# AaronWatters/contourist

Measured on AMD Instinct MI355X. Metric: Mvoxels/s isosurface extraction on 512^3 fp32 grid, higher is better.
Workload: dtype f32

## Files before the change

### contourist_amd/csrc/cx_api.hip

```cpp
#include <cmath>
#include <cstdio>
#include <cstring>
#include <new>
#include <string>

#include "cx_ctx.h"

static int fail(cx_ctx* ctx, int code, const char* msg) {
    if (ctx) ctx->err = msg;
    return code;
}

extern "C" const char* cx_version(void) { return "contourist_hip gfx950 " __DATE__; }

extern "C" int cx_ctx_create(int device_id, cx_ctx** out) {
    if (!out) return CX_ERR_INVALID;
    *out = nullptr;
    int ndev = 0;
    if (hipGetDeviceCount(&ndev) != hipSuccess || device_id < 0 || device_id >= ndev) return CX_ERR_HIP;
    cx_ctx* ctx = new (std::nothrow) cx_ctx();
    if (!ctx) return CX_ERR_NOMEM;
    ctx->device = device_id;
    if (hipSetDevice(device_id) != hipSuccess || hipStreamCreate(&ctx->stream) != hipSuccess) {
        delete ctx;
        return CX_ERR_HIP;
    }
    ctx->own_stream = ctx->stream;
    if (ctx->counters.grow(ctx, 2048) != CX_OK ||
        hipHostMalloc(&ctx->counters_host, 2 * CX_CNT_WORDS * sizeof(uint32_t)) != hipSuccess) {
        cx_ctx_destroy(ctx);
        return CX_ERR_NOMEM;
    }
    *out = ctx;
    return CX_OK;
}

extern "C" int cx_ctx_destroy(cx_ctx* ctx) {
    if (!ctx) return CX_OK;
    (void)hipSetDevice(ctx->device);
    (void)hipDeviceSynchronize();
    cx_rccl_comm_free(ctx);
    cx_levels_free(ctx);
    cx_xfer_free(ctx);
    cx_post_free(ctx);
    cx_comp_free(ctx);
    cx_topo_free(ctx);
    cx_simplify_free(ctx);
    cx_clip_free(ctx);
    cx_cap_free(ctx);
    cx_pick_free(ctx);
    cx_state4_free(ctx);
    cx_state2_free(ctx);
    if (ctx->counters_host) (void)hipHostFree(ctx->counters_host);
    for (auto& ev : ctx->events)
        for (int n = 0; n < 5; n++)
            if (ev.e[n]) (void)hipEventDestroy(ev.e[n]);
    if (ctx->own_stream) (void)hipStreamDestroy(ctx->own_stream);
    delete ctx;
    return CX_OK;
}

extern "C" int cx_device_bytes(cx_ctx* ctx, int64_t* live_bytes, int64_t* allocations) {
    if (live_bytes) *live_bytes = ctx ? ctx->tally.live_bytes : cx_process_tally.live_bytes.load();
    if (allocations) *allocations = ctx ? ctx->tally.allocations : cx_process_tally.allocations.load();
    return CX_OK;
}

extern "C" const char* cx_last_error(cx_ctx* ctx) { return ctx ? ctx->err.c_str() : "null context"; }

extern "C" int cx_set_stream(cx_ctx* ctx, void* hip_stream) {
    if (!ctx) return CX_ERR_INVALID;
    ctx->stream = hip_stream ? (hipStream_t)hip_stream : ctx->own_stream;
    return CX_OK;
}

extern "C" int cx_synchronize(cx_ctx* ctx) {
    if (!ctx) return CX_ERR_INVALID;
    CX_HIP(ctx, hipSetDevice(ctx->device));
    CX_HIP(ctx, hipStreamSynchronize(ctx->stream));
    return CX_OK;
}

static int set_grid_dims(cx_ctx* ctx, int64_t n0, int64_t n1, int64_t n2) {
    if (n0 < 2 || n1 < 2 || n2 < 2) return fail(ctx, CX_ERR_INVALID, "grid must have at least 2 samples per axis");
    const int64_t N = n0 * n1 * n2;
    if (N > (1LL << 29)) return fail(ctx, CX_ERR_UNSUPPORTED, "more than 2^29 samples in one grid: partition into slabs");
// ... 213 lines not shown
        P.tq = nullptr; P.tlimit = 0;
        if (!fused && !typed && cx_debug_knob("CX_TQ", 0u)) {
            if ((rc = ctx->tq.grow(ctx, Z.need))) return rc;
            P.tq = ctx->tq; P.tlimit = T.wcap;
        }
        P.write_records = (!fused && !tiled && !cx_debug_knob("CX_K2_ENTRIES", 0u)) ? CX_RECORDS_SLIM : CX_RECORDS_NONE;
        if (P.write_records == CX_RECORDS_SLIM) {
            if ((rc = ctx->cbase.grow(ctx, (size_t)ctx->ccap() / 64u + 1u))) return rc;
            P.cbase = ctx->cbase;
        }
        if (tiled) {
            P.qa = nullptr;
            if ((rc = ctx->fj.grow(ctx, (size_t)P.n0 * (4u * T.njg) * P.n2 + 64u))) return rc;
            if ((rc = ctx->fk.grow(ctx, (size_t)P.n0 * P.n1 * (2u * T.nks) + 64u))) return rc;
            if ((rc = ctx->bnd.grow(ctx, (size_t)T.nblocks * 2u * T.bndcap))) return rc;
            if ((rc = ctx->bndn.grow(ctx, (size_t)T.nblocks * 2u))) return rc;
            if ((rc = ctx->torder.grow(ctx, (size_t)T.nblocks * 6u))) return rc;
            P.fj = ctx->fj; P.fk = ctx->fk; P.bnd = ctx->bnd; P.bndn = ctx->bndn; P.torder = ctx->torder;
            P.tile_cap = cx_debug_knob("CX_TILE_CAP", cx_tile_cap_default());
        }
        P.nvw = cx_vertex_stage_waves(P);
        if ((rc = ctx->rstart.grow(ctx, (size_t)P.nvw + 1u))) return rc;
        P.rstart = ctx->rstart;
        P.nkw = cx_triangle_stage_waves(P);
        if ((rc = ctx->kstart.grow(ctx, (size_t)P.nkw + 1u))) return rc;
        P.kstart = ctx->kstart;
        ctx->last = P;
    }
    ctx->last_task = T;
    ctx->last_flags = flags;
    ctx->path = staged ? (fused ? 2 : (tiled ? 3 : 1)) : 0;
    ctx->records_valid = staged ? (P.write_records == CX_RECORDS_FULL) : true;
    cx_ctx::evset* ev = nullptr;
    if (ctx->timing && ctx->nevents < (int)(sizeof(ctx->events) / sizeof(ctx->events[0])) && ctx->events[ctx->nevents].e[4])
        ev = &ctx->events[ctx->nevents++];
    if (!staged)
        CX_HIP(ctx, hipMemsetAsync(ctx->counters, 0, CX_CNT_WORDS * sizeof(uint32_t), ctx->stream));
    if (ev) CX_HIP(ctx, hipEventRecord(ev->e[0], ctx->stream));
    if (staged) {
        cx_launch_stream(P, T, ctx->stream);
        if (ev) CX_HIP(ctx, hipEventRecord(ev->e[1], ctx->stream));
        cx_launch_scan_waves(P, T, ctx->stream);
        if (ev) CX_HIP(ctx, hipEventRecord(ev->e[2], ctx->stream));
        if (fused) cx_launch_emit_mesh(P, T, ctx->stream);
        else if (tiled) cx_launch_tile_emit(P, T, ctx->hash_xy, ctx->stream);
        else cx_launch_emit_vertices(P, T, ctx->stream);
    } else {
        cx_launch_classify_generic(P, ctx->stream);
        if (ev) CX_HIP(ctx, hipEventRecord(ev->e[1], ctx->stream));
        if (ev) CX_HIP(ctx, hipEventRecord(ev->e[2], ctx->stream));
    }
    if (ev) CX_HIP(ctx, hipEventRecord(ev->e[3], ctx->stream));
    if (!fused && !tiled) {
        if (staged && P.write_records) cx_launch_emit_triangles_q(P, T, ctx->hash_xy, ctx->stream);
        else if (staged) cx_launch_emit_triangles_e(P, T, ctx->hash_xy, ctx->stream);
        else cx_launch_emit_triangles(P, ctx->hash_xy, ctx->stream);
    }
    if (ev) CX_HIP(ctx, hipEventRecord(ev->e[4], ctx->stream));
    CX_HIP(ctx, hipGetLastError());
    ctx->extracted = true;
    ctx->counts_fetched = false;
    ctx->post_valid = false;
    ctx->keep_valid = false;
    ctx->cap_valid = false;
    cx_levels_invalidate(ctx);
    return CX_OK;
}

// ... 170 lines not shown
    hipLaunchKernelGGL(cx_k_read_bw, dim3(256 * 8), dim3(256), 0, ctx->stream, static_cast<const uint4*>(device_ptr), n16, sink);
    CX_HIP(ctx, hipGetLastError());
    double best = 0.0;
    const uint32_t grids[3] = {256u * 8u, 256u * 16u, 256u * 32u};
    for (int r = 0; r < reps; r++)
        for (uint32_t g : grids) {
            CX_HIP(ctx, hipEventRecord(e0, ctx->stream));
            hipLaunchKernelGGL(cx_k_read_bw, dim3(g), dim3(256), 0, ctx->stream, static_cast<const uint4*>(device_ptr), n16, sink);
            CX_HIP(ctx, hipGetLastError());
            CX_HIP(ctx, hipEventRecord(e1, ctx->stream));
            CX_HIP(ctx, hipEventSynchronize(e1));
            float ms = 0.f;
            CX_HIP(ctx, hipEventElapsedTime(&ms, e0, e1));
            if (ms > 0.f) best = fmax(best, (double)n16 * 16.0 / (ms * 1e-3) / 1e9);
        }
    *out_GBps = best;
    return CX_OK;
}
extern "C" int cx_measure_read_bandwidth(cx_ctx* ctx, const void* device_ptr, int64_t bytes, int reps, double* out_GBps) {
    if (!ctx || !device_ptr || bytes < (1 << 20) || reps < 1 || !out_GBps) return ctx ? fail(ctx, CX_ERR_INVALID, "cx_measure_read_bandwidth: bad argument") : CX_ERR_INVALID;
    CX_HIP(ctx, hipSetDevice(ctx->device));
    if (!ctx->counters) return fail(ctx, CX_ERR_STATE, "context has no scratch words yet (extract once first)");
    cx_buf<uint32_t> sink;
    hipEvent_t e0 = nullptr, e1 = nullptr;
    int rc = sink.grow(ctx, 256);
    if (!rc && (hipEventCreate(&e0) != hipSuccess || hipEventCreate(&e1) != hipSuccess)) rc = fail(ctx, CX_ERR_HIP, "cx_measure_read_bandwidth: hipEventCreate failed");
    if (!rc) rc = read_bandwidth(ctx, device_ptr, (size_t)bytes / 16u, reps, e0, e1, sink, out_GBps);
    if (rc) (void)hipStreamSynchronize(ctx->stream);
    if (e0) (void)hipEventDestroy(e0);
    if (e1) (void)hipEventDestroy(e1);
    return rc;
}

extern "C" int cx_timing_enable(cx_ctx* ctx, int on) {
    if (!ctx) return CX_ERR_INVALID;
    ctx->nevents = 0;
    ctx->timing = false;
    if (!on) return CX_OK;
    CX_HIP(ctx, hipSetDevice(ctx->device));
    for (auto& ev : ctx->events)
        for (int n = 0; n < 5; n++)
            if (!ev.e[n]) CX_HIP(ctx, hipEventCreateWithFlags(&ev.e[n], hipEventDisableSystemFence));
    ctx->timing = true;
    return CX_OK;
}

extern "C" int cx_timing_read(cx_ctx* ctx, double ms[8], int* n) {
    if (!ctx || !ms) return CX_ERR_INVALID;
    CX_HIP(ctx, hipSetDevice(ctx->device));
    CX_HIP(ctx, hipStreamSynchronize(ctx->stream));
    for (int k = 0; k < 8; k++) ms[k] = 0.0;
    for (int i = 0; i < ctx->nevents; i++) {
        float d[4] = {0, 0, 0, 0};
        for (int k = 0; k < 4; k++) CX_HIP(ctx, hipEventElapsedTime(&d[k], ctx->events[i].e[k], ctx->events[i].e[k + 1]));
        ms[0] += d[0] + d[1] + d[2]; ms[1] += d[3]; ms[2] += d[0] + d[1] + d[2] + d[3];
        ms[3] += d[0]; ms[4] += d[1]; ms[5] += d[2];
    }
    if (n) *n = ctx->nevents;
    ctx->nevents = 0;
    return CX_OK;
}
```

### contourist_amd/csrc/cx_common.h

```cpp
#pragma once
#include <hip/hip_runtime.h>
#include <stdint.h>

#include <type_traits>

#include "../../include/contourist_hip.h"
#include "cx_tables.h"

#include <cstdlib>
#include <cstring>
static inline bool cx_debug_enabled() {
    static const bool on = [] { const char* e = getenv("CX_DEBUG"); return e && strcmp(e, "1") == 0; }();
    return on;
}
static inline uint32_t cx_debug_knob(const char* name, uint32_t dflt) {
    if (!cx_debug_enabled()) return dflt;
    const char* e = getenv(name);
    return (e && atoi(e) > 0) ? (uint32_t)atoi(e) : dflt;
}

struct cx_fdiv {
    uint32_t mul, sh1, sh2, d;
};

// ... 39 lines not shown
template <> struct cx_dt<CX_DTYPE_U8> : cx_dt_int<CX_DTYPE_U8, uint8_t> {};
template <> struct cx_dt<CX_DTYPE_I8> : cx_dt_int<CX_DTYPE_I8, int8_t> {};
template <> struct cx_dt<CX_DTYPE_U16> : cx_dt_int<CX_DTYPE_U16, uint16_t> {};
template <> struct cx_dt<CX_DTYPE_I16> : cx_dt_int<CX_DTYPE_I16, int16_t> {};
template <> struct cx_dt<CX_DTYPE_F16> : cx_dt_narrow<CX_DTYPE_F16, uint16_t, uint16_t> {
    static __device__ __forceinline__ float cvt(uint32_t v) { return (float)__builtin_bit_cast(_Float16, (uint16_t)v); }
};
template <> struct cx_dt<CX_DTYPE_BF16> : cx_dt_narrow<CX_DTYPE_BF16, uint16_t, uint16_t> {
    static __device__ __forceinline__ float cvt(uint32_t v) { return __uint_as_float(v << 16); }
};
template <int DT>
__device__ __forceinline__ const typename cx_dt<DT>::T* cx_grid_data(const cx_grid_ref& g) {
    return static_cast<const typename cx_dt<DT>::T*>(g.p);
}
template <int DT>
__device__ __forceinline__ float cx_sample(const cx_grid_ref& g, size_t i) {
    if constexpr (DT == CX_DTYPE_F32) return cx_grid_data<DT>(g)[i];
    else return cx_dt<DT>::cvt((uint32_t)(typename cx_dt<DT>::bits)cx_grid_data<DT>(g)[i]);
}
static inline size_t cx_dtype_size(int32_t dt) {
    return dt == CX_DTYPE_F32 ? 4u : (dt == CX_DTYPE_U8 || dt == CX_DTYPE_I8) ? 1u : 2u;
}
static inline bool cx_dtype_valid(int32_t dt) { return dt >= CX_DTYPE_F32 && dt <= CX_DTYPE_BF16; }
#define CX_DISPATCH_DTYPE(dt, F)                                   \
    switch (dt) {                                                  \
        case CX_DTYPE_U8: F(CX_DTYPE_U8); break;                   \
        case CX_DTYPE_I8: F(CX_DTYPE_I8); break;                   \
        case CX_DTYPE_U16: F(CX_DTYPE_U16); break;                 \
        case CX_DTYPE_I16: F(CX_DTYPE_I16); break;                 \
        case CX_DTYPE_F16: F(CX_DTYPE_F16); break;                 \
        case CX_DTYPE_BF16: F(CX_DTYPE_BF16); break;               \
        default: F(CX_DTYPE_F32); break;                           \
    }

struct cx_params {
    cx_grid_ref grid;
    uint32_t n0, n1, n2;
    uint32_t nsamples;
    cx_fdiv div_plane;
    cx_fdiv div_row;
    float vcmp;
    float near_abs;
    float vhi, vlo;
    double value;
    double tol_value;
    uint32_t flags;
    uint32_t org0, org1, org2;
    uint64_t* celltab;
    cx_vrec* verts;
    uint4* cells;
    int32_t* tris;
    uint32_t vcap, ccap, tcap;
    uint32_t* counters;
    unsigned long long* stamps;
    uint32_t* queue;
    struct cx_brec* brec;
    struct cx_wsum* wsum;
    struct cx_wbase* wbase;
    struct cx_bdesc* flat;
    uint32_t fcap;
    uint32_t* qa;
    uint32_t* info;
    const uint8_t* hbytes;
    uint64_t* info64;
    cx_fdiv div_ci;
    uint32_t* chunksum;
    uint32_t fused;
    uint32_t* rstart;
    uint32_t nvw;
    uint32_t qlimit;
    uint32_t* kstart;
    uint32_t nkw;
    uint32_t write_records;
    uint32_t records_only;
    uint2* cbase;
    float* tq;
    uint32_t tlimit;
    uint64_t* fj;
    uint64_t* fk;
    uint4* bnd;
    uint32_t* bndn;
    uint32_t* torder;
    uint32_t tile_cap;
};
enum { CX_RECORDS_NONE = 0, CX_RECORDS_FULL = 1, CX_RECORDS_SLIM = 2 };
#ifndef CX_SWP
#define CX_SWP 16u
#endif

struct cx_wsum {
    uint32_t nb;
    uint32_t v, t, c, b;
    uint32_t nq;
    uint32_t near;
    uint32_t nr;
};
struct cx_wbase {
    uint32_t v, t, c, boff;
};
struct cx_brec {
    uint32_t qoff, n, vpre, tpre, cpre, near, pad0, pad1;
};

struct cx_bdesc {
    uint32_t w;
    uint32_t qofs, n;
    uint32_t vbase, tbase, cbase;
    uint32_t near;
    uint32_t rbase;
    uint32_t p, j0, k0;
    uint32_t nsteps;
};

struct cx_task {
    uint32_t ci;
    uint32_t nks, njg, nic;
// ... 41 lines not shown
```

### contourist_amd/csrc/cx_ctx.h

```cpp
#pragma once
#include <atomic>
#include <string>
#include <type_traits>
#include <utility>

#include "cx_common.h"

#define CX_HIP(ctx, call)                                                                        \
    do {                                                                                         \
        hipError_t e__ = (call);                                                                 \
        if (e__ != hipSuccess) {                                                                 \
            (ctx)->err = std::string(#call) + ": " + hipGetErrorString(e__);                     \
            return (e__ == hipErrorOutOfMemory) ? CX_ERR_NOMEM : CX_ERR_HIP;                      \
        }                                                                                        \
    } while (0)

static inline uint32_t cx_blocks(size_t n, uint32_t b = 256) { return (uint32_t)((n + b - 1) / b); }
static inline dim3 cx_grid1(size_t n) { return dim3(n ? cx_blocks(n) : 1u); }
static inline unsigned long long cx_table_size(size_t n) {
    unsigned long long s = 1024;
    while (s < 2 * (unsigned long long)n + 16) s <<= 1;
    return s;
}

// ... 103 lines not shown
    cx_buf<uint32_t> counters;
    uint32_t* counters_host = nullptr;
    bool extracted = false;
    bool counts_fetched = false;
    cx_counts counts = {0, 0, 0, 0};
    cx_params last;
    cx_buf<uint8_t> tri_keep;
    cx_buf<uint8_t> seed_buf[8];
    int seed_mode = 0;
    bool keep_valid = false;
    cx_buf<float4> attr_n0;
    cx_buf<double> attr_n1;
    cx_buf<float> attr_v0;
    cx_buf<double> attr_v1;
    cx_buf<uint8_t> attr_e1;
    cx_buf<uint8_t> attr_grid;
    cx_buf<float4> attr_c0;
    cx_buf<double> attr_c1;
    struct cx_comp_state* comp = nullptr;
    struct cx_simplify_state* simp = nullptr;
    struct cx_topo_state* topo = nullptr;
    struct cx_clip_state* clip = nullptr;
    struct cx_cap_state* cap = nullptr;
    bool cap_valid = false;
    struct cx_pick_state* pick = nullptr;
    cx_post_state* post = nullptr;
    bool post_valid = false;
    cx_buf<unsigned long long> stamps;
    void* rccl_comm = nullptr;
    bool rccl_owned = true;
    int rccl_rank = 0, rccl_world = 1;
    void* xfer_stage[2] = {nullptr, nullptr};
    hipEvent_t xfer_ev[2] = {nullptr, nullptr};
    struct evset { hipEvent_t e[5] = {nullptr, nullptr, nullptr, nullptr, nullptr}; };
    bool timing = false;
    int nevents = 0;
    evset events[256];
};

template <typename T>
int cx_buf<T>::fail(cx_ctx* ctx, size_t bytes, hipError_t e) {
    ctx->err = std::string("device buffer (") + std::to_string(bytes) + " bytes): " + hipGetErrorString(e);
    return (e == hipErrorOutOfMemory) ? CX_ERR_NOMEM : CX_ERR_HIP;
}
template <typename T>
hipError_t cx_buf<T>::alloc(cx_ctx* ctx, size_t n) {
    void* fresh = nullptr;
    const hipError_t e = hipMalloc(&fresh, n * sizeof(T));
    if (e != hipSuccess) return e;
    p_ = static_cast<T*>(fresh); cap_ = n; tally_ = &ctx->tally;
    tally_->live_bytes += (int64_t)bytes(); tally_->allocations++;
    cx_process_tally.live_bytes += (int64_t)bytes(); cx_process_tally.allocations++;
    return hipSuccess;
}
template <typename T>
int cx_buf<T>::grow(cx_ctx* ctx, size_t need) {
    if (cap_ >= need && p_) return CX_OK;
    if (need == 0) return CX_OK;
    hipError_t e = hipStreamSynchronize(ctx->stream);
    if (e == hipSuccess && p_) e = hipFree(p_);
    forget();
    if (e == hipSuccess) e = alloc(ctx, need);
    return e == hipSuccess ? CX_OK : fail(ctx, need * sizeof(T), e);
}
template <typename T>
int cx_buf<T>::grow_keep(cx_ctx* ctx, size_t used, size_t need) {
    if (cap_ >= need && p_) return CX_OK;
    if (need == 0) return CX_OK;
    const size_t want = need > cap_ + cap_ / 2 ? need : cap_ + cap_ / 2;
    cx_buf fresh;
// ... 101 lines not shown
```

### contourist_amd/csrc/cx_stream3d.h

```cpp
#pragma once

__device__ __forceinline__ uint32_t cx_task_of_block(const cx_task& T) {
    return (blockIdx.x & 7u) * T.chunk + (blockIdx.x >> 3);
}
struct cx_tile {
    uint32_t k0, j0, p, ib, nrows;
};
__device__ __forceinline__ cx_tile cx_tile_of(const cx_params& P, const cx_task& T, uint32_t b, uint32_t wave) {
    cx_tile t;
    const uint32_t ks = b % T.nks; b /= T.nks;
    const uint32_t jg = b % T.njg;
    const uint32_t ic = b / T.njg;
    t.k0 = ks * 256u;
    t.j0 = jg * (4u * CX_RJ) + wave * CX_RJ;
    t.p = ic * T.ci;
    t.ib = min(t.p + T.ci, P.n0);
    t.nrows = (t.j0 < P.n1) ? min((uint32_t)CX_RJ, P.n1 - t.j0) : 0u;
    return t;
}

#define CX_SQ 512u
#define CX_PLW 260u
#define CX_SBR 32u
static_assert((CX_SWP - 1u) * 1024u / CX_BATCH_MIN + 1u <= CX_SBR, "a streaming wave can close more batches than its LDS stage holds");
static_assert(CX_SQ >= 512u, "half a wave's lanes queue up to 512 cells per step");
template <int DT> struct cx_row4 { typedef float4 v; typedef float h; };
template <> struct cx_row4<CX_DTYPE_U8> { typedef uint32_t v; typedef uint32_t h; };
template <> struct cx_row4<CX_DTYPE_I8> { typedef uint32_t v; typedef uint32_t h; };
template <> struct cx_row4<CX_DTYPE_U16> { typedef cx_v2u v; typedef uint32_t h; };
template <> struct cx_row4<CX_DTYPE_I16> { typedef cx_v2u v; typedef uint32_t h; };
template <> struct cx_row4<CX_DTYPE_F16> { typedef cx_v2u v; typedef uint32_t h; };
template <> struct cx_row4<CX_DTYPE_BF16> { typedef cx_v2u v; typedef uint32_t h; };
template <typename V, size_t AL>
struct __attribute__((packed, aligned(AL))) cx_row4_ua { V v; };
template <int DT>
__device__ __forceinline__ void cx_row4_unpack(const typename cx_row4<DT>::v& w, float& x, float& y, float& z, float& t) {
    if constexpr (sizeof(typename cx_dt<DT>::T) == 1) {
        x = cx_dt<DT>::cvt(w); y = cx_dt<DT>::cvt(w >> 8); z = cx_dt<DT>::cvt(w >> 16); t = cx_dt<DT>::cvt(w >> 24);
    } else {
        x = cx_dt<DT>::cvt(w.x); y = cx_dt<DT>::cvt(w.x >> 16); z = cx_dt<DT>::cvt(w.y); t = cx_dt<DT>::cvt(w.y >> 16);
    }
}
template <bool ALIGNED, int DT>
__device__ __forceinline__ void cx_stream_tile(const cx_params& P, const cx_task& T, const uint32_t b) {
    __shared__ uint32_t s_q[4][CX_SQ];
    __shared__ uint32_t s_br[4][CX_SBR][5];
    extern __shared__ __attribute__((aligned(16))) float s_pl_dyn[];
    __shared__ uint32_t s_tot[4][8];
    __shared__ uint8_t s_ntri[256];
    if (b >= T.nblocks) return;
    s_ntri[threadIdx.x] = cx_d_voxel_ntri[threadIdx.x];
    if (b == 0u && threadIdx.x < 3u && P.torder) P.counters[CX_CNT_TCLS + threadIdx.x] = 0u;
    __syncthreads();
    const uint32_t lane = cx_lane_id();
    const uint32_t wave = __builtin_amdgcn_readfirstlane(threadIdx.x >> 6);
    uint32_t* q = s_q[wave];
    uint32_t ql = 0, qflushed = 0;
    uint32_t nbl = 0, nbflushed = 0;
    const uint32_t w = b * 4u + wave;
    unsigned long long* stamp = P.stamps ? P.stamps + (size_t)w * 4u : nullptr;
    if (stamp && lane == 0) stamp[0] = __builtin_amdgcn_s_memtime();
    const cx_tile tile = cx_tile_of(P, T, b, wave);
    const uint32_t k0 = tile.k0, j0 = tile.j0, ib = tile.ib, nrows = tile.nrows;
    uint32_t p = tile.p;
    uint32_t* __restrict__ gq = P.queue + (size_t)w * T.wcap;
    cx_brec* __restrict__ brec = P.brec + (size_t)w * T.bcap;
    const typename cx_dt<DT>::bits* __restrict__ A = reinterpret_cast<const typename cx_dt<DT>::bits*>(cx_grid_data<DT>(P.grid));
    cx_cnt acc = {0, 0, 0, 0};
    uint32_t qn = 0, qstart = 0, nb = 0;
    uint32_t rv = 0, rt = 0, rc = 0;
    uint32_t nr = 0;
    uint32_t tv = 0;
    bool overflow_t = false;
    float dnear = 3.0e38f;
    cx_fast_geom G;
    G.pstart = p; G.j0 = j0; G.k0 = k0;
    bool overflow = false;
// ... 241 lines not shown
    if (near && qn != 0u && !overflow) {
        __threadfence();
        cx_run ex = {0, 0, 0, 0, 0};
        cx_process_queue<false, DT>(P, [&](uint32_t x) { return cx_entry_lin(P, G, __builtin_nontemporal_load(gq + x)); }, qn, lane, false, ex, nullptr);
        really_near = !(ex.v == rv && ex.t == rt && ex.c == rc && ex.s == 0u);
        run.b = ex.b;
        if (really_near) { run.v = ex.v; run.t = ex.t; run.c = ex.c; }
    }
    if (overflow_t && qn != 0u && !overflow) really_near = true;
    if (really_near) {
        nb = 1;
        nr = (qn + 63u) >> 6;
        if (lane == 0) {
            cx_brec R;
            R.qoff = 0; R.n = qn; R.vpre = 0; R.tpre = 0; R.cpre = 0; R.near = 1; R.pad0 = 0; R.pad1 = 0;
            brec[0] = R;
        }
    }
    if (lane == 0) {
        cx_wsum S;
        S.nb = nb; S.v = run.v; S.t = run.t; S.c = run.c; S.b = run.b; S.nq = qn; S.near = really_near ? 1u : 0u; S.nr = nr;
        P.wsum[w] = S;
        s_tot[wave][0] = run.v; s_tot[wave][1] = run.t; s_tot[wave][2] = run.c; s_tot[wave][3] = run.b; s_tot[wave][4] = nb;
        s_tot[wave][5] = (really_near && qn != 0u) ? 1u : 0u;
        s_tot[wave][6] = nr;
        s_tot[wave][7] = overflow ? 1u : 0u;
    }
    __syncthreads();
    if (threadIdx.x < 8u) {
        const uint32_t sum = s_tot[0][threadIdx.x] + s_tot[1][threadIdx.x] + s_tot[2][threadIdx.x] + s_tot[3][threadIdx.x];
        uint32_t* cs = P.chunksum + (size_t)(b >> 6) * 8u;
        if (sum) atomicAdd(cs + threadIdx.x, sum);
    }
}
template <bool ALIGNED, int DT>
__global__ __launch_bounds__(256, CX_K1_MIN_WAVES) void cx_k_stream(const cx_params P, const cx_task T) {
    cx_stream_tile<ALIGNED, DT>(P, T, cx_task_of_block(T));
}
#define CX_LEVELS_PER_LAUNCH 8u
struct cx_params_pack {
    cx_params p[CX_LEVELS_PER_LAUNCH];
};
template <bool ALIGNED, int DT>
__global__ __launch_bounds__(256, CX_K1_MIN_WAVES) void cx_k_stream_levels(const cx_params_pack LP, const cx_task T, const uint32_t nlevels) {
    const uint32_t seq = blockIdx.x >> 3;
    const uint32_t tile_seq = seq / nlevels, level = seq - tile_seq * nlevels;
    cx_stream_tile<ALIGNED, DT>(LP.p[level], T, (blockIdx.x & 7u) * T.chunk + tile_seq);
}

__device__ __forceinline__ void cx_scan_list_chunk(const cx_params& P, const cx_task& T, const uint32_t nw, const uint32_t g, const uint32_t nchunks) {
    __shared__ uint32_t s_part[4][8];
    __shared__ uint32_t s_own[4][6];
    const uint32_t tid = threadIdx.x, lane = cx_lane_id(), wave = tid >> 6;
    uint32_t acc[6] = {0, 0, 0, 0, 0, 0}, near_any = 0, rall = 0, over_any = 0;
    for (uint32_t c = tid; c < nchunks; c += 256u) {
        const uint4 lo = *reinterpret_cast<const uint4*>(P.chunksum + (size_t)c * 8u);
        const uint4 hi = *reinterpret_cast<const uint4*>(P.chunksum + (size_t)c * 8u + 4u);
        if (c < g) { acc[0] += lo.x; acc[1] += lo.y; acc[2] += lo.z; acc[3] += lo.w; acc[4] += hi.x; acc[5] += hi.z; }
        near_any |= hi.y;
        rall += hi.z;
        over_any |= hi.w;
    }
    const uint32_t w = g * 256u + tid;
    cx_wsum S;
    S.nb = S.v = S.t = S.c = S.b = S.nq = S.near = S.nr = 0;
    if (w < nw) S = P.wsum[w];
    near_any |= (S.near != 0u && S.nq != 0u) ? 1u : 0u;
    const uint32_t x[6] = {S.v, S.t, S.c, S.b, S.nb, S.nr};
    uint32_t inc[6];
#pragma unroll
    for (int m = 0; m < 6; m++) {
        inc[m] = cx_wave_incl_scan(x[m], lane);
        const uint32_t before = cxd_wave_add(acc[m]);
        if (lane == 63u) { s_own[wave][m] = inc[m]; s_part[wave][m] = before; }
    }
    {
        const uint32_t nr = (__ballot(near_any != 0u) != 0ULL) ? 1u : 0u;
        const uint32_t ra = cxd_wave_add(rall);
        const uint32_t ov = (__ballot(over_any != 0u) != 0ULL) ? 1u : 0u;
        if (lane == 63u) { s_part[wave][6] = nr | (ov << 1); s_part[wave][7] = ra; }
// ... 37 lines not shown
        uint32_t rank = 0;
#pragma unroll
        for (uint32_t c = 0; c < 3u; c++) {
            const uint64_t m = __ballot(cls == c);
            if (cls == c) rank = cx_mbcnt(m);
            if (lane == 0) s_cls[c][wave] = (uint32_t)__popcll(m);
        }
        __syncthreads();
        if (tid < 3u) {
            const uint32_t n = s_cls[tid][0] + s_cls[tid][1] + s_cls[tid][2] + s_cls[tid][3];
            s_clsbase[tid] = n ? atomicAdd(&P.counters[CX_CNT_TCLS + tid], n) : 0u;
        }
        __syncthreads();
        if (cls < 3u) {
            uint32_t at = s_clsbase[cls] + rank;
            for (uint32_t ww = 0; ww < wave; ww++) at += s_cls[cls][ww];
            P.torder[(size_t)cls * (nw >> 1) + at] = w >> 1;
        } else if (cls == 3u) {
            P.bndn[w >> 1] = 0u;
        }
    }
    if (g == nchunks - 1u && tid == 255u) {
        P.counters[CX_CNT_VERTS] = ex[0] + x[0]; P.counters[CX_CNT_TRIS] = ex[1] + x[1];
        P.counters[CX_CNT_CELLS] = ex[2] + x[2]; P.counters[CX_CNT_BORDER] = ex[3] + x[3];
        P.counters[CX_CNT_BATCHES] = ex[4] + x[4];
        P.counters[CX_CNT_ROUNDS] = rounds;
        const uint32_t fl = s_part[0][6] | s_part[1][6] | s_part[2][6] | s_part[3][6];
        P.counters[CX_CNT_NEAR] = fl & 1u;
        P.counters[CX_CNT_OVERFLOW] = (fl >> 1) & 1u;
        P.counters[CX_CNT_TILEOVF] = 0u;
    }
}
__global__ __launch_bounds__(256) void cx_k_scan_list(const cx_params P, const cx_task T, const uint32_t nw) {
    cx_scan_list_chunk(P, T, nw, blockIdx.x, gridDim.x);
}
__global__ __launch_bounds__(256) void cx_k_scan_list_levels(const cx_params* __restrict__ LP, const cx_task T, const uint32_t nw) {
    const cx_params P = LP[blockIdx.y];
    cx_scan_list_chunk(P, T, nw, blockIdx.x, gridDim.x);
}
```

### contourist_amd/csrc/cx_tri3d.h

```cpp
#pragma once

#define CX_PY_P1 11400714785074694791ULL
#define CX_PY_P2 14029467366897019727ULL
#define CX_PY_P5 2870177450012600261ULL
__device__ __forceinline__ uint64_t py_round(uint64_t acc, uint32_t x) {
    acc += (uint64_t)x * CX_PY_P2;
    acc = (acc << 31) | (acc >> 33);
    return acc * CX_PY_P1;
}
__device__ __forceinline__ uint64_t py_round_signed(uint64_t acc, int32_t x) {
    const uint64_t lane = (x == -1) ? ~1ULL : (uint64_t)(int64_t)x;
    acc += lane * CX_PY_P2;
    acc = (acc << 31) | (acc >> 33);
    return acc * CX_PY_P1;
}
__device__ __forceinline__ uint64_t py_round_tail(uint64_t acc) {
    acc = (acc << 31) | (acc >> 33);
    return acc * CX_PY_P1;
}
__device__ __forceinline__ uint64_t py_finish3(uint64_t acc) {
    acc += 3ULL ^ (CX_PY_P5 ^ 3527539ULL);
    return (acc == ~0ULL) ? 1546275796ULL : acc;
}
__global__ void cx_k_hash_xy(uint64_t* table, uint32_t n0, uint32_t n1, uint32_t org0, uint32_t org1) {
// ... 459 lines not shown
    for (uint32_t c = 0; c < 6; c++) {
        uint2 pr = make_uint2(0u, 0u);
        if ((A.geo >> c) & 1u) {
            const uint32_t qa = A.qa[c];
            const uint32_t below = qa & ((1u << bit[c]) - 1u);
            const uint32_t at = qb[c] + (qa >> 16) + __popc(below);
            const uint64_t e = P.info64[at];
            pr = make_uint2((uint32_t)e, (uint32_t)(e >> 32));
        }
        I.nb[c] = pr;
    }
    I.ck = A.ck;
    I.hb[0] = I.hb[1] = I.hb[2] = I.hb[3] = 0;
    I.hxy[0] = I.hxy[1] = I.hxy[2] = I.hxy[3] = 0;
    const uint32_t sm = A.rec.y & 0xFFu, tetskip = (A.rec.y >> 8) & 0x3Fu, ntri = (A.rec.y >> 16) & 0xFFu;
    if ((P.flags & CX_DIAG_CPYTHON310) && cx_need_hash(sm, tetskip, ntri) != 0u) {
        struct __attribute__((packed, aligned(8))) u64x2 { uint64_t a, b; };
        const u64x2 p0 = *reinterpret_cast<const u64x2*>(hash_xy + A.ij);
        const u64x2 p1 = *reinterpret_cast<const u64x2*>(hash_xy + (A.ij + P.n1));
        I.hxy[0] = p0.a; I.hxy[1] = p0.b; I.hxy[2] = p1.a; I.hxy[3] = p1.b;
    }
}
__device__ __forceinline__ void cx_triq_pin2(cx_tri_in& I) {
    asm volatile("" : "+v"(I.hxy[0]), "+v"(I.hxy[1]), "+v"(I.hxy[2]), "+v"(I.hxy[3]) :: "memory");
    asm volatile("" : "+v"(I.nb[0].x), "+v"(I.nb[0].y), "+v"(I.nb[1].x), "+v"(I.nb[1].y), "+v"(I.nb[2].x), "+v"(I.nb[2].y) :: "memory");
    asm volatile("" : "+v"(I.nb[3].x), "+v"(I.nb[3].y), "+v"(I.nb[4].x), "+v"(I.nb[4].y), "+v"(I.nb[5].x), "+v"(I.nb[5].y) :: "memory");
}
#ifndef CX_K2Q_MIN_WAVES
#define CX_K2Q_MIN_WAVES 5
#endif
template <bool NEG_ORIGIN, bool SLIM>
__global__ __launch_bounds__(256, CX_K2Q_MIN_WAVES) void cx_k_emit_triangles_q(const cx_params P, const cx_task T, const uint64_t* __restrict__ hash_xy) {
    __shared__ cx_tri_lds L;
    const uint32_t ncells = min(P.counters[CX_CNT_CELLS], P.ccap);
    if (P.counters[CX_CNT_TRIS] > P.tcap || P.counters[CX_CNT_VERTS] > P.vcap) return;
    if (SLIM && P.counters[CX_CNT_CELLS] > P.ccap) return;
    if (blockIdx.x * blockDim.x >= ncells) return;
    cx_tri_lds_init(L);
    __syncthreads();
    const uint32_t lane = cx_lane_id();
    const uint32_t wave = __builtin_amdgcn_readfirstlane(threadIdx.x >> 6);
    const uint32_t stride = gridDim.x * blockDim.x;
    uint32_t idx = blockIdx.x * blockDim.x + threadIdx.x;
    const uint4 zero = make_uint4(0, 0, 0, 0);
    auto record = [&](uint32_t at) {
        const uint32_t c = min(at, ncells - 1u);
        if constexpr (SLIM) {
            const uint2 r = cx_load_record2(reinterpret_cast<const uint2*>(P.cells) + c);
            const uint2 b = P.cbase[__builtin_amdgcn_readfirstlane(c >> 6)];
            return make_uint4(r.x, r.y, b.x, b.y);
        } else {
            return cx_load_record(P.cells + c);
        }
    };
    auto valid = [&](const uint4& r, uint32_t at) { return (at < ncells) ? r : zero; };
    cx_tri_qa Ab, Ac;
    cx_tri_in Ia, Ib;
    uint4 rec_c = record(idx + 2u * stride);
    {
        uint4 r0 = record(idx), r1 = record(idx + stride);
        asm volatile("" : "+v"(r0.x), "+v"(r0.y), "+v"(r0.z), "+v"(r0.w), "+v"(r1.x), "+v"(r1.y), "+v"(r1.z), "+v"(r1.w) :: "memory");
        cx_triq_stage1(P, T, L, valid(r0, idx), Ac);
        cx_triq_stage1(P, T, L, valid(r1, idx + stride), Ab);
        cx_triq_pin1(Ac, rec_c);
        cx_triq_pin1(Ab, rec_c);
        cx_triq_stage2(P, T, hash_xy, Ac, Ia);
        cx_triq_pin2(Ia);
    }
    while (idx - lane < ncells) {
        const uint32_t nidx = idx + stride;
        uint4 rec_d = record(nidx + 2u * stride);
        cx_triq_stage1(P, T, L, valid(rec_c, nidx + stride), Ac);
        cx_triq_stage2(P, T, hash_xy, Ab, Ib);
        const uint32_t ttot = cx_tri_phase1<NEG_ORIGIN, SLIM>(P, L, lane, wave, Ia);
        cx_tri_phase2(P, L, lane, wave, ttot);
        cx_triq_pin1(Ac, rec_d);
        cx_triq_pin2(Ib);
        Ia = Ib;
        Ab = Ac;
        rec_c = rec_d;
        idx = nidx;
    }
}

__device__ __forceinline__ cx_bdesc cx_desc_uniform(const cx_bdesc& D) {
    cx_bdesc U;
    U.w = __builtin_amdgcn_readfirstlane(D.w); U.qofs = __builtin_amdgcn_readfirstlane(D.qofs); U.n = __builtin_amdgcn_readfirstlane(D.n);
    U.vbase = 0; U.cbase = 0; U.p = 0; U.j0 = 0; U.k0 = 0; U.nsteps = 0;
    U.tbase = __builtin_amdgcn_readfirstlane(D.tbase);
    U.near = __builtin_amdgcn_readfirstlane(D.near); U.rbase = __builtin_amdgcn_readfirstlane(D.rbase);
    return U;
}
struct cx_esrc {
    uint32_t f, nbatches, lo, hi;
    uint32_t at, bend;
    uint32_t qofs, w;
    uint32_t bend_round;
    uint32_t tbase;
    cx_bdesc next;
    bool done;
};
__device__ __forceinline__ void cx_esrc_enter(const cx_params& P, cx_esrc& S, const cx_bdesc& Draw) {
    const cx_bdesc D = cx_desc_uniform(Draw);
    const uint32_t nrb = (D.n + 63u) >> 6;
    const uint32_t r0 = max(S.lo, D.rbase) - D.rbase, r1 = min(S.hi, D.rbase + nrb) - D.rbase;
    S.qofs = D.qofs; S.w = D.w; S.bend_round = D.rbase + nrb; S.tbase = D.tbase;
    if (D.near) { S.at = 0u; S.bend = (r0 == 0u) ? D.n : 0u; }
    else { S.at = r0 * 64u; S.bend = min(D.n, r1 * 64u); }
    if (S.f + 1u < S.nbatches) S.next = P.flat[S.f + 1u];
}
__device__ __forceinline__ void cx_esrc_advance(const cx_params& P, cx_esrc& S) {
    while (S.at >= S.bend && !S.done) {
        if (S.bend_round >= S.hi || S.f + 1u >= S.nbatches) { S.done = true; break; }
        S.f++;
        cx_esrc_enter(P, S, S.next);
// ... 114 lines not shown
```

### contourist_amd/csrc/cx_vertex3d.h

```cpp
#pragma once

__device__ __forceinline__ void cx_skip_rounds(const cx_params& P, const cx_fast_geom& G, const uint32_t* q, uint32_t rounds, uint32_t lane,
                                               const uint8_t* ntri_lut, cx_run& run) {
    uint32_t v = 0, t = 0, c = 0;
    for (uint32_t r = 0; r < rounds; r++) {
        const uint32_t e = q[r * 64u + lane];
        uint32_t i, j, k;
        cx_decode_entry(P, G, e, i, j, k);
        const uint32_t vm = cx_corner_valid(P, i, j, k);
        const uint32_t sm = cx_entry_signs(e);
        const uint32_t s0 = (sm & 1u) ? 0xFFu : 0u;
        const uint32_t nv = __popc(((sm ^ s0) & vm) & 0xFEu);
        const uint32_t nt = (vm == 0xFFu) ? (uint32_t)ntri_lut[sm] : 0u;
        v += nv; t += nt; c += (nv | nt) ? 1u : 0u;
    }
    run.v += cxd_wave_add(v); run.t += cxd_wave_add(t); run.c += cxd_wave_add(c);
}

#ifndef CX_S3_MIN_WAVES
#define CX_S3_MIN_WAVES 1
#endif
template <bool TQ, int DT>
__global__ __launch_bounds__(256, CX_S3_MIN_WAVES) void cx_k_emit_vertices(const cx_params P, const cx_task T) {
    __shared__ float4 s_vstage[4][CX_VSTAGE_LDS];
    __shared__ uint8_t s_ntri[256];
    s_ntri[threadIdx.x] = cx_d_voxel_ntri[threadIdx.x];
    __syncthreads();
    const uint32_t lane = cx_lane_id();
    const uint32_t wave = __builtin_amdgcn_readfirstlane(threadIdx.x >> 6);
    const uint32_t nbatches = min(P.counters[CX_CNT_BATCHES], P.fcap);
    const uint32_t rounds = P.counters[CX_CNT_ROUNDS];
    const uint32_t nvw = gridDim.x * 4u;
    const uint32_t share = max((rounds + nvw - 1u) / nvw, CX_S3_MIN_SHARE);
    const uint32_t lo = (blockIdx.x * 4u + wave) * share;
    if (lo >= rounds || nbatches == 0u) return;
    const uint32_t hi = min(rounds, lo + share);
    uint32_t f = P.rstart[blockIdx.x * 4u + wave];
    if (f >= nbatches) return;
    cx_bdesc D = P.flat[f];
    for (;;) {
        const uint32_t fn = f + 1u;
        cx_bdesc Dn = D;
        if (fn < nbatches) Dn = P.flat[fn];
        const uint32_t nrb = (D.n + 63u) >> 6;
        const uint32_t r0 = max(lo, D.rbase) - D.rbase, r1 = min(hi, D.rbase + nrb) - D.rbase;
        cx_fast_geom G;
        G.pstart = D.p; G.j0 = D.j0; G.k0 = D.k0;
        const uint32_t* __restrict__ q = P.queue + D.qofs;
        cx_run run;
        run.v = D.vbase; run.t = D.tbase; run.c = D.cbase; run.b = 0;
        uint64_t* __restrict__ info = P.info64 + D.qofs;
        if (!D.near) {
            if (r0) cx_skip_rounds(P, G, q, r0, lane, s_ntri, run);
            if (TQ)
                cx_emit_queue_t(P, G, q, r0 * 64u, min(D.n, r1 * 64u), lane, run, reinterpret_cast<uint32_t*>(s_vstage[wave]), s_ntri, info,
                                reinterpret_cast<const uint32_t*>(P.tq) + ((size_t)D.w * T.wcap) - __builtin_amdgcn_readfirstlane(P.wbase[D.w].v));
            else
                cx_emit_queue_fast<DT>(P, G, q, r0 * 64u, min(D.n, r1 * 64u), lane, run, reinterpret_cast<uint32_t*>(s_vstage[wave]), s_ntri, info);
        } else if (r0 == 0u) {
            cx_process_queue<true, DT>(P, [&](uint32_t x) { return cx_entry_lin(P, G, q[x]); }, D.n, lane, true, run, reinterpret_cast<cx_vrec*>(s_vstage[wave]), info);
        }
        if (D.rbase + nrb >= hi || fn >= nbatches) break;
        f = fn;
        D = Dn;
    }
}
```

Measured before the change: 440,700.

## Time kernels with in-kernel realtime stamps and use scalar loads for vertex setup

After: 440,700 (median of 2 runs). No clear change (+0.0%).

```diff
diff --git a/contourist_amd/csrc/cx_api.hip b/contourist_amd/csrc/cx_api.hip
--- a/contourist_amd/csrc/cx_api.hip
+++ b/contourist_amd/csrc/cx_api.hip
@@ -52,6 +52,7 @@
     cx_state4_free(ctx);
     cx_state2_free(ctx);
     if (ctx->counters_host) (void)hipHostFree(ctx->counters_host);
+    if (ctx->tslots_host) (void)hipHostFree(ctx->tslots_host);
     for (auto& ev : ctx->events)
         for (int n = 0; n < 5; n++)
             if (ev.e[n]) (void)hipEventDestroy(ev.e[n]);
@@ -331,8 +332,13 @@
     ctx->path = staged ? (fused ? 2 : (tiled ? 3 : 1)) : 0;
     ctx->records_valid = staged ? (P.write_records == CX_RECORDS_FULL) : true;
     cx_ctx::evset* ev = nullptr;
-    if (ctx->timing && ctx->nevents < (int)(sizeof(ctx->events) / sizeof(ctx->events[0])) && ctx->events[ctx->nevents].e[4])
-        ev = &ctx->events[ctx->nevents++];
+    if (ctx->timing && ctx->nevents < (int)cx_ctx::CX_TIMED_MAX && ctx->tslots && ctx->events[ctx->nevents].e[4]) {
+        const bool stamped = staged && P.write_records == CX_RECORDS_SLIM && !cx_debug_knob("CX_TIMING_EVENTS", 0u);
+        const int i = ctx->nevents++;
+        ctx->by_events[i] = !stamped;
+        if (stamped) P.tslots = ctx->tslots + (size_t)i * CX_TS_KERNELS;
+        else ev = &ctx->events[i];
+    }
     if (!staged)
         CX_HIP(ctx, hipMemsetAsync(ctx->counters, 0, CX_CNT_WORDS * sizeof(uint32_t), ctx->stream));
     if (ev) CX_HIP(ctx, hipEventRecord(ev->e[0], ctx->stream));
@@ -569,12 +575,32 @@
     return rc;
 }
 
+static int timing_clear_used(cx_ctx* ctx) {
+    if (ctx->nevents > 0 && ctx->tslots)
+        CX_HIP(ctx, hipMemsetAsync(ctx->tslots, 0, (size_t)ctx->nevents * CX_TS_KERNELS * sizeof(cx_tslot), ctx->stream));
+    ctx->nevents = 0;
+    return CX_OK;
+}
+
 extern "C" int cx_timing_enable(cx_ctx* ctx, int on) {
     if (!ctx) return CX_ERR_INVALID;
-    ctx->nevents = 0;
+    CX_HIP(ctx, hipSetDevice(ctx->device));
     ctx->timing = false;
+    {
+        const int rc = timing_clear_used(ctx);
+        if (rc) return rc;
+    }
     if (!on) return CX_OK;
-    CX_HIP(ctx, hipSetDevice(ctx->device));
+    if (!ctx->tslots) {
+        const size_t nslots = (size_t)cx_ctx::CX_TIMED_MAX * CX_TS_KERNELS;
+        const int rc = ctx->tslots.grow(ctx, nslots);
+        if (rc) return rc;
+        CX_HIP(ctx, hipMemsetAsync(ctx->tslots, 0, ctx->tslots.bytes(), ctx->stream));
+        CX_HIP(ctx, hipHostMalloc(&ctx->tslots_host, nslots * sizeof(cx_tslot)));
+        int khz = 0;
+        if (hipDeviceGetAttribute(&khz, hipDeviceAttributeWallClockRate, ctx->device) != hipSuccess || khz <= 0) khz = 100000;
+        ctx->ticks_per_ms = (double)khz;
+    }
     for (auto& ev : ctx->events)
         for (int n = 0; n < 5; n++)
             if (!ev.e[n]) CX_HIP(ctx, hipEventCreateWithFlags(&ev.e[n], hipEventDisableSystemFence));
@@ -582,18 +608,39 @@
     return CX_OK;
 }
 
+static double stamp_ms(const cx_tslot& S, double ticks_per_ms) {
+    unsigned long long end = 0ULL;
+    for (uint32_t k = 0; k < CX_TS_ENDS; k++) end = S.end[k] > end ? S.end[k] : end;
+    if (S.start == 0ULL || end <= S.start) return 0.0;
+    return (double)(end - S.start) / ticks_per_ms;
+}
+
 extern "C" int cx_timing_read(cx_ctx* ctx, double ms[8], int* n) {
     if (!ctx || !ms) return CX_ERR_INVALID;
     CX_HIP(ctx, hipSetDevice(ctx->device));
     CX_HIP(ctx, hipStreamSynchronize(ctx->stream));
     for (int k = 0; k < 8; k++) ms[k] = 0.0;
+    bool stamps = false;
+    for (int i = 0; i < ctx->nevents; i++) stamps = stamps || !ctx->by_events[i];
+    if (stamps) {
+        CX_HIP(ctx, hipMemcpyAsync(ctx->tslots_host, ctx->tslots, (size_t)ctx->nevents * CX_TS_KERNELS * sizeof(cx_tslot), hipMemcpyDeviceToHost, ctx->stream));
+        CX_HIP(ctx, hipStreamSynchronize(ctx->stream));
+    }
     for (int i = 0; i < ctx->nevents; i++) {
-        float d[4] = {0, 0, 0, 0};
-        for (int k = 0; k < 4; k++) CX_HIP(ctx, hipEventElapsedTime(&d[k], ctx->events[i].e[k], ctx->events[i].e[k + 1]));
-        ms[0] += d[0] + d[1] + d[2]; ms[1] += d[3]; ms[2] += d[0] + d[1] + d[2] + d[3];
-        ms[3] += d[0]; ms[4] += d[1]; ms[5] += d[2];
-    }
+        double d[4] = {0, 0, 0, 0};
+        if (ctx->by_events[i]) {
+            float e[4] = {0, 0, 0, 0};
+            for (int k = 0; k < 4; k++) CX_HIP(ctx, hipEventElapsedTime(&e[k], ctx->events[i].e[k], ctx->events[i].e[k + 1]));
+            for (int k = 0; k < 4; k++) d[k] = e[k];
+        } else {
+            const cx_tslot* S = ctx->tslots_host + (size_t)i * CX_TS_KERNELS;
+            d[0] = stamp_ms(S[CX_TS_STREAM], ctx->ticks_per_ms); d[1] = stamp_ms(S[CX_TS_SCAN], ctx->ticks_per_ms);
+            d[2] = stamp_ms(S[CX_TS_VERTS], ctx->ticks_per_ms); d[3] = stamp_ms(S[CX_TS_TRIS], ctx->ticks_per_ms);
+        }
+        ms[3] += d[0]; ms[4] += d[1]; ms[5] += d[2]; ms[1] += d[3];
+    }
+    ms[0] = ms[3] + ms[4] + ms[5];
+    ms[2] = ms[0] + ms[1];
     if (n) *n = ctx->nevents;
-    ctx->nevents = 0;
-    return CX_OK;
-}
+    return timing_clear_used(ctx);
+}
diff --git a/contourist_amd/csrc/cx_common.h b/contourist_amd/csrc/cx_common.h
--- a/contourist_amd/csrc/cx_common.h
+++ b/contourist_amd/csrc/cx_common.h
@@ -95,6 +95,41 @@
         case CX_DTYPE_BF16: F(CX_DTYPE_BF16); break;               \
         default: F(CX_DTYPE_F32); break;                           \
     }
+
+#define CX_TS_ENDS 32u
+struct cx_tslot {
+    unsigned long long start;
+    unsigned long long end[CX_TS_ENDS];
+};
+enum { CX_TS_STREAM = 0, CX_TS_SCAN = 1, CX_TS_VERTS = 2, CX_TS_TRIS = 3, CX_TS_KERNELS = 4 };
+typedef unsigned long long cx_ts_stash[2];
+__device__ __forceinline__ void cx_ts_begin(cx_tslot* ts, uint32_t k, unsigned long long* stash) {
+    unsigned long long end = 0ULL, t0 = 0ULL;
+    if (ts) {
+        end = (unsigned long long)reinterpret_cast<uintptr_t>(&ts[k].end[blockIdx.x & (CX_TS_ENDS - 1u)]);
+        if (blockIdx.x == 0u) t0 = __builtin_amdgcn_s_memrealtime();
+    }
+    if (threadIdx.x == 0u) { stash[0] = end; stash[1] = t0; }
+}
+__device__ __forceinline__ void cx_ts_end(const unsigned long long* stash) {
+    if (!stash || (threadIdx.x & 63u) != 0u) return;
+    typedef __attribute__((address_space(1))) unsigned long long gu64;
+    gu64* const end = reinterpret_cast<gu64*>((uintptr_t)stash[0]);
+    if (!end) return;
+    __hip_atomic_fetch_max(end, (unsigned long long)__builtin_amdgcn_s_memrealtime(), __ATOMIC_RELAXED, __HIP_MEMORY_SCOPE_AGENT);
+    if (threadIdx.x == 0u && stash[1] != 0ULL) end[-1] = stash[1];
+}
+template <typename T>
+__device__ __forceinline__ T cx_ro(const T* p) {
+    static_assert(sizeof(T) % 4u == 0u && std::is_trivially_copyable<T>::value, "words");
+    const __attribute__((address_space(4))) uint32_t* q = (const __attribute__((address_space(4))) uint32_t*)(p);
+    uint32_t w[sizeof(T) / 4u];
+#pragma unroll
+    for (uint32_t k = 0; k < sizeof(T) / 4u; k++) w[k] = q[k];
+    T v;
+    __builtin_memcpy(&v, w, sizeof(T));
+    return v;
+}
 
 struct cx_params {
     cx_grid_ref grid;
@@ -145,6 +180,7 @@
     uint32_t* bndn;
     uint32_t* torder;
     uint32_t tile_cap;
+    cx_tslot* tslots;
 };
 enum { CX_RECORDS_NONE = 0, CX_RECORDS_FULL = 1, CX_RECORDS_SLIM = 2 };
 #ifndef CX_SWP
diff --git a/contourist_amd/csrc/cx_ctx.h b/contourist_amd/csrc/cx_ctx.h
--- a/contourist_amd/csrc/cx_ctx.h
+++ b/contourist_amd/csrc/cx_ctx.h
@@ -159,10 +159,15 @@
     int rccl_rank = 0, rccl_world = 1;
     void* xfer_stage[2] = {nullptr, nullptr};
     hipEvent_t xfer_ev[2] = {nullptr, nullptr};
+    enum { CX_TIMED_MAX = 256 };
     struct evset { hipEvent_t e[5] = {nullptr, nullptr, nullptr, nullptr, nullptr}; };
     bool timing = false;
     int nevents = 0;
-    evset events[256];
+    evset events[CX_TIMED_MAX];
+    bool by_events[CX_TIMED_MAX] = {};
+    cx_buf<cx_tslot> tslots;
+    cx_tslot* tslots_host = nullptr;
+    double ticks_per_ms = 1.0e5;
 };
 
 template <typename T>
diff --git a/contourist_amd/csrc/cx_stream3d.h b/contourist_amd/csrc/cx_stream3d.h
--- a/contourist_amd/csrc/cx_stream3d.h
+++ b/contourist_amd/csrc/cx_stream3d.h
@@ -42,7 +42,7 @@
     }
 }
 template <bool ALIGNED, int DT>
-__device__ __forceinline__ void cx_stream_tile(const cx_params& P, const cx_task& T, const uint32_t b) {
+__device__ __forceinline__ void cx_stream_tile(const cx_params& P, const cx_task& T, const uint32_t b, const unsigned long long* ts_stash) {
     __shared__ uint32_t s_q[4][CX_SQ];
     __shared__ uint32_t s_br[4][CX_SBR][5];
     extern __shared__ __attribute__((aligned(16))) float s_pl_dyn[];
@@ -350,10 +350,13 @@
         uint32_t* cs = P.chunksum + (size_t)(b >> 6) * 8u;
         if (sum) atomicAdd(cs + threadIdx.x, sum);
     }
+    cx_ts_end(ts_stash);
 }
 template <bool ALIGNED, int DT>
 __global__ __launch_bounds__(256, CX_K1_MIN_WAVES) void cx_k_stream(const cx_params P, const cx_task T) {
-    cx_stream_tile<ALIGNED, DT>(P, T, cx_task_of_block(T));
+    __shared__ cx_ts_stash s_ts;
+    cx_ts_begin(P.tslots, CX_TS_STREAM, s_ts);
+    cx_stream_tile<ALIGNED, DT>(P, T, cx_task_of_block(T), s_ts);
 }
 #define CX_LEVELS_PER_LAUNCH 8u
 struct cx_params_pack {
@@ -363,7 +366,7 @@
 __global__ __launch_bounds__(256, CX_K1_MIN_WAVES) void cx_k_stream_levels(const cx_params_pack LP, const cx_task T, const uint32_t nlevels) {
     const uint32_t seq = blockIdx.x >> 3;
     const uint32_t tile_seq = seq / nlevels, level = seq - tile_seq * nlevels;
-    cx_stream_tile<ALIGNED, DT>(LP.p[level], T, (blockIdx.x & 7u) * T.chunk + tile_seq);
+    cx_stream_tile<ALIGNED, DT>(LP.p[level], T, (blockIdx.x & 7u) * T.chunk + tile_seq, nullptr);
 }
 
 __device__ __forceinline__ void cx_scan_list_chunk(const cx_params& P, const cx_task& T, const uint32_t nw, const uint32_t g, const uint32_t nchunks) {
@@ -467,7 +470,10 @@
     }
 }
 __global__ __launch_bounds__(256) void cx_k_scan_list(const cx_params P, const cx_task T, const uint32_t nw) {
+    __shared__ cx_ts_stash s_ts;
+    cx_ts_begin(P.tslots, CX_TS_SCAN, s_ts);
     cx_scan_list_chunk(P, T, nw, blockIdx.x, gridDim.x);
+    cx_ts_end(s_ts);
 }
 __global__ __launch_bounds__(256) void cx_k_scan_list_levels(const cx_params* __restrict__ LP, const cx_task T, const uint32_t nw) {
     const cx_params P = LP[blockIdx.y];
diff --git a/contourist_amd/csrc/cx_tri3d.h b/contourist_amd/csrc/cx_tri3d.h
--- a/contourist_amd/csrc/cx_tri3d.h
+++ b/contourist_amd/csrc/cx_tri3d.h
@@ -515,6 +515,8 @@
 template <bool NEG_ORIGIN, bool SLIM>
 __global__ __launch_bounds__(256, CX_K2Q_MIN_WAVES) void cx_k_emit_triangles_q(const cx_params P, const cx_task T, const uint64_t* __restrict__ hash_xy) {
     __shared__ cx_tri_lds L;
+    __shared__ cx_ts_stash s_ts;
+    cx_ts_begin(P.tslots, CX_TS_TRIS, s_ts);
     const uint32_t ncells = min(P.counters[CX_CNT_CELLS], P.ccap);
     if (P.counters[CX_CNT_TRIS] > P.tcap || P.counters[CX_CNT_VERTS] > P.vcap) return;
     if (SLIM && P.counters[CX_CNT_CELLS] > P.ccap) return;
@@ -564,6 +566,7 @@
         rec_c = rec_d;
         idx = nidx;
     }
+    cx_ts_end(s_ts);
 }
 
 __device__ __forceinline__ cx_bdesc cx_desc_uniform(const cx_bdesc& D) {
diff --git a/contourist_amd/csrc/cx_vertex3d.h b/contourist_amd/csrc/cx_vertex3d.h
--- a/contourist_amd/csrc/cx_vertex3d.h
+++ b/contourist_amd/csrc/cx_vertex3d.h
@@ -24,20 +24,22 @@
 __global__ __launch_bounds__(256, CX_S3_MIN_WAVES) void cx_k_emit_vertices(const cx_params P, const cx_task T) {
     __shared__ float4 s_vstage[4][CX_VSTAGE_LDS];
     __shared__ uint8_t s_ntri[256];
+    __shared__ cx_ts_stash s_ts;
+    cx_ts_begin(P.tslots, CX_TS_VERTS, s_ts);
     s_ntri[threadIdx.x] = cx_d_voxel_ntri[threadIdx.x];
     __syncthreads();
     const uint32_t lane = cx_lane_id();
     const uint32_t wave = __builtin_amdgcn_readfirstlane(threadIdx.x >> 6);
-    const uint32_t nbatches = min(P.counters[CX_CNT_BATCHES], P.fcap);
-    const uint32_t rounds = P.counters[CX_CNT_ROUNDS];
+    const uint32_t nbatches = min(cx_ro(P.counters + CX_CNT_BATCHES), P.fcap);
+    const uint32_t rounds = cx_ro(P.counters + CX_CNT_ROUNDS);
     const uint32_t nvw = gridDim.x * 4u;
     const uint32_t share = max((rounds + nvw - 1u) / nvw, CX_S3_MIN_SHARE);
     const uint32_t lo = (blockIdx.x * 4u + wave) * share;
     if (lo >= rounds || nbatches == 0u) return;
     const uint32_t hi = min(rounds, lo + share);
-    uint32_t f = P.rstart[blockIdx.x * 4u + wave];
+    uint32_t f = cx_ro(P.rstart + (blockIdx.x * 4u + wave));
     if (f >= nbatches) return;
-    cx_bdesc D = P.flat[f];
+    cx_bdesc D = cx_ro(P.flat + f);
     for (;;) {
         const uint32_t fn = f + 1u;
         cx_bdesc Dn = D;
@@ -64,4 +66,5 @@
         f = fn;
         D = Dn;
     }
+    cx_ts_end(s_ts);
 }
```
